# HanGuo97/flute

Hardware: AMD Instinct MI355X
Metric: qgemm effective GB/s, M=1, W4G64 NF4 fp16, K=N=4096 (Llama-3-8B linear), HBM-cold (higher is better)
Workload: dtype f16

## Files before the change

### flute_amd/csrc/qgemm_fast.h

```cpp
#pragma once
#include "qgemm_oneshot.h"

namespace flute_amd {

__host__ __device__ constexpr size_t fast_lds_bytes(int W, int KW, int D, int lg, int mb = 1) {
    return (size_t)65536 + (size_t)mb * 512 * D * KW * 2 + (size_t)W * 4 * D * (512 >> lg) * 2 + 128 + (size_t)W * 64;
}

struct FastRing { int R, GS; };
__host__ __device__ constexpr FastRing fast_ring_of(int opt) {
    constexpr FastRing rings[] = {{3, 8}, {2, 8}, {3, 8}, {4, 4}, {5, 4}, {3, 6}, {4, 5}};
    return rings[(opt >> 6) & 7];
}

template <typename T, int MB, int D, int R, int GS>
__device__ __forceinline__ void fast_pieces(ring16_t (&q)[D][1], uint32_t x_lane, uint32_t x_row, uint32_t s_lane, uint32_t s_piece,
                                            uint32_t lane_off, float (&acc)[4][MB]) {
    using NT = Num<T>;
    constexpr int NL = 16 * D;
    constexpr int NGR = (NL + GS - 1) / GS;
    static_assert(R >= 2 && GS >= 1 && GS <= 16, "lookup ring");
    auto younger = [](int g) constexpr {
        const int last = (g + R - 1 < NGR - 1) ? g + R - 1 : NGR - 1;
        const int end = ((last + 1) * GS < NL) ? (last + 1) * GS : NL;
        return end - (g + 1) * GS > 0 ? end - (g + 1) * GS : 0;
    };
    static_assert((R - 1) * GS <= 16, "at most one read of over-wait: lgkmcnt encodes 0 .. 15");
    ring16_t xq[D][MB];
    u32x2_t sq[D];
    uint32_t lv[NL];
    float al[4][MB];
#pragma unroll
    for (int i = 0; i < D; ++i)
#pragma unroll
        for (int m = 0; m < MB; ++m) xq[i][m] = lds_hidden128(x_lane + ((uint32_t)i << 10) + (uint32_t)m * x_row);
#pragma unroll
    for (int i = 0; i < D; ++i) sq[i] = lds_hidden64(s_lane + (uint32_t)i * s_piece);

    auto issue_group = [&](auto g_tag) {
        constexpr int g = decltype(g_tag)::value;
        constexpr int L0 = g * GS, L1 = (L0 + GS < NL) ? L0 + GS : NL;
        static_for<L1 - L0>([&](auto n_tag) {
            constexpr int L = L0 + decltype(n_tag)::value;
            if constexpr (L % 16 == 0) vm_wait_regs<D - 1 - L / 16>(q[L / 16][0]);
        });
        uint32_t ad[GS];
#pragma unroll
        for (int n = 0; n < L1 - L0; ++n) {
            const int L = L0 + n;
            ad[n] = __builtin_amdgcn_perm(q[L / 16][0][(L % 16) / 4], lane_off, 0x0c0c0400u | ((4u + (uint32_t)(L % 4)) << 8));
        }
#pragma unroll
        for (int n = 0; n < L1 - L0; ++n) { uint32_t& r = ad[n]; asm volatile("" : "+v"(r)); }
#pragma unroll
        for (int n = 0; n < L1 - L0; ++n) lv[L0 + n] = lds_lookup32(ad[n]);
    };
    auto wait_group = [&](auto g_tag) {
        constexpr int g = decltype(g_tag)::value;
        constexpr int L0 = g * GS, L1 = (L0 + GS < NL) ? L0 + GS : NL;
        constexpr int YOUNGER = younger(g);
        static_assert(YOUNGER <= 16, "over-wait");
        asm volatile("s_waitcnt lgkmcnt(%0)" : : "n"(YOUNGER < 15 ? YOUNGER : 15) : "memory");
#pragma unroll
        for (int n = L0; n < L1; ++n) { uint32_t& r = lv[n]; asm volatile("" : "+v"(r) : : "memory"); }
        if constexpr (g == 0) {
#pragma unroll
            for (int i = 0; i < D; ++i) {
#pragma unroll
                for (int m = 0; m < MB; ++m) { ring16_t& r = xq[i][m]; asm volatile("" : "+v"(r) : : "memory"); }
                u32x2_t& s2 = sq[i];
                asm volatile("" : "+v"(s2) : : "memory");
            }
        }
    };

    static_for<(R - 1 < NGR ? R - 1 : NGR)>([&](auto g_tag) { issue_group(g_tag); });
    static_for<NGR>([&](auto g_tag) {
        constexpr int g = decltype(g_tag)::value;
        constexpr int L0 = g * GS, L1 = (L0 + GS < NL) ? L0 + GS : NL;
        if constexpr (g + R - 1 < NGR) issue_group(std::integral_constant<int, g + R - 1>{});
        wait_group(g_tag);
#pragma unroll
        for (int L = L0; L < L1; ++L) {
            const int I = L / 16, ww = (L % 16) / 4, j = L % 4;
#pragma unroll
            for (int m = 0; m < MB; ++m) {
                if (ww == 0) al[j][m] = NT::dot2z(lv[L], xq[I][m][ww]);
                else al[j][m] = NT::dot2(lv[L], xq[I][m][ww], al[j][m]);
            }
            if (ww == 3) {
                const uint32_t w = sq[I][j / 2];
                const float sf = scale_to_float<T>((j & 1) ? (w >> 16) : (w & 0xffffu));
#pragma unroll
                for (int m = 0; m < MB; ++m) acc[j][m] = __builtin_fmaf(al[j][m], sf, acc[j][m]);
            }
        }
    });
}

template <typename T, int TILEP, int W, int KW, int D, int MB = 1, int OPT = 0>
__global__ __launch_bounds__(W * 64) void qgemv_fast_kernel(
    const uint32_t* __restrict__ Qp, const void* __restrict__ Sp, const void* __restrict__ Ap,
    const uint32_t* __restrict__ QM2, void* __restrict__ Dp, int N, int lg, int M,
    uint64_t* __restrict__ stamps) {
    using NT = Num<T>;
    constexpr int K = 512 * D * KW;
    constexpr bool POW2 = (D & (D - 1)) == 0;
    constexpr int LK = ilog2_c(K);
    constexpr int UPW = W / KW;
    constexpr int ENT = 256 / W;
    constexpr int RUNS = 32 / W;
    constexpr int XP = MB * K / 8;
    constexpr int XPR = (XP + W * 64 - 1) / (W * 64);
    constexpr int NSL = (2 * D * 8 + 63) / 64;
    constexpr uint32_t X_BASE = 65536u;
    constexpr uint32_t S_BASE = X_BASE + (uint32_t)MB * K * 2u;
    static_assert(W == 4 || W == 8 || W == 16, "waves per workgroup");
    static_assert(MB == 1 || MB == 2 || MB == 4, "rows per pass");
    static_assert((KW & (KW - 1)) == 0 && D >= 1 && D <= 8 && W % KW == 0, "K split: a power of two; 1 .. 8 pieces per wave");
    static_assert(MB * K * 2 <= 32768, "activation rows");

    extern __shared__ __attribute__((aligned(16))) char smem[];
    if (lds_base_of(smem) != 0) __builtin_trap();
#ifdef FLUTE_STAMPS
    uint64_t stamp[16];
    for (int i = 0; i < 16; ++i) stamp[i] = 0;
    stamp[0] = wall_clock64();
    stamp[1] = __builtin_amdgcn_s_memtime();
#define FLUTE_FSTAMP(i) stamp[i] = __builtin_amdgcn_s_memtime()
#else
#define FLUTE_FSTAMP(i)
#endif
    const int tid = threadIdx.x;
    const int lane = tid & 63;
    const int wave = __builtin_amdgcn_readfirstlane(tid >> 6);
    const uint32_t lane16 = (uint32_t)lane * 16u;
    const int gpp = 512 >> lg;
    const uint32_t red_base = S_BASE + (uint32_t)(W * 4 * D * gpp * 2);
    const int ul = wave / KW, kpart = wave % KW;
    const int unit = blockIdx.x * UPW + ul;
    const int col0 = (unit / TILEP) * (4 * TILEP) + (unit % TILEP);

    const srd_t lut_srd = make_srd(QM2, 1024u);
    uint32_t lut_v = buf_load4((uint32_t)(wave * ENT + (lane & (ENT - 1))) * 4u, lut_srd);
    const srd_t x_srd = make_srd(Ap, (uint32_t)M * (uint32_t)K * 2u);
    ring16_t xv[XPR];
#pragma unroll
    for (int r = 0; r < XPR; ++r) {
        const int pidx = (r * W + wave) * 64 + lane;
        xv[r] = buf_load16((XP % (W * 64) == 0 || pidx < XP) ? (uint32_t)pidx * 16u : 0x80000000u, x_srd, 0);
    }
    const int lgh = (8 + ilog2_c(D)) - lg;
    const int lG = LK - lg;
    const int G = K >> lg;
    const int gpw2 = (D * (512 >> lg)) >> 1;
    auto col_of = [&](int q) { return POW2 ? (q >> lgh) : (lg == 6 ? q / (D * 4) : (lg == 7 ? q / (D * 2) : q / D)); };
    const srd_t s_srd = make_srd(Sp, (uint32_t)((size_t)N * (size_t)G * 2));
    uint32_t sv[NSL];
#pragma unroll
    for (int r = 0; r < NSL; ++r) {
        const int q = lane + 64 * r;
        const int j = col_of(q);
        const int gp = POW2 ? (q & ((1 << lgh) - 1)) : (q - j * gpw2);
        const uint32_t vo = POW2 ? (uint32_t)((((col0 + j * TILEP) << lG) + (kpart << (lgh + 1)) + 2 * gp) * 2)
                                 : (uint32_t)(((col0 + j * TILEP) * G + kpart * 2 * gpw2 + 2 * gp) * 2);
        sv[r] = buf_load4_at(j < 4 ? vo : 0x80000000u, s_srd, 0);
    }
    const srd_t q_srd = make_srd(Qp + (size_t)unit * (K / 2), (uint32_t)K * 2u);
    ring16_t q[D][1];
    static_for<D>([&](auto i_tag) {
        constexpr int i = decltype(i_tag)::value;
        const uint32_t vo = lane16 + (uint32_t)(kpart * D + i) * 1024u;
        if constexpr (OPT & 1) q[i][0] = buf_load16(vo, q_srd, 0);
        else q[i][0] = buf_load16_nt(vo, q_srd, 0);
    });
    __builtin_amdgcn_sched_barrier(0);
    FLUTE_FSTAMP(2);

    vm_wait_regs<XPR + NSL + D>(lut_v);
    FLUTE_FSTAMP(3);
    {
        uint32_t te[RUNS];
#pragma unroll
        for (int u = 0; u < RUNS; ++u) te[u] = (uint32_t)__builtin_amdgcn_ds_bpermute((u * 8 + (lane >> 3)) * 4, (int)lut_v);
#pragma unroll
        for (int u = 0; u < RUNS; ++u) {
            const uint32_t addr = (uint32_t)(wave * ENT + u * 8 + (lane >> 3)) * 256u + (uint32_t)(lane & 7) * 16u;
            *reinterpret_cast<uint4*>(smem + addr) = make_uint4(te[u], te[u], te[u], te[u]);
        }
    }
    FLUTE_FSTAMP(4);
    if (KW > 1 && wave == 0 && lane < UPW) *reinterpret_cast<int*>(smem + red_base + lane * 4) = 0;
    static_for<XPR>([&](auto r_tag) {
        constexpr int r = decltype(r_tag)::value;
        vm_wait_regs<XPR - 1 - r + NSL + D>(xv[r]);
        if constexpr (r == 0) { FLUTE_FSTAMP(5); }
        const int pidx = (r * W + wave) * 64 + lane;
        if (XP % (W * 64) == 0 || pidx < XP) {
            *reinterpret_cast<uint4*>(smem + X_BASE + (uint32_t)pidx * 16u) = make_uint4(xv[r].x, xv[r].y, xv[r].z, xv[r].w);
        }
    });
    FLUTE_FSTAMP(6);
    asm volatile("s_waitcnt lgkmcnt(0)" ::: "memory");
    __builtin_amdgcn_s_barrier();
    FLUTE_FSTAMP(7);

    const uint32_t sbase = S_BASE + (uint32_t)(wave * 4 * D * gpp * 2);
#pragma unroll
    for (int r = 0; r < NSL; ++r) {
        vm_wait_regs<D>(sv[r]);
        const int qq = lane + 64 * r;
        const int j = col_of(qq);
        const int gp = POW2 ? (qq & ((1 << lgh) - 1)) : (qq - j * gpw2);
        if (j < 4) {
            uint16_t* img = reinterpret_cast<uint16_t*>(smem + sbase) + (2 * gp) * 4 + j;
            img[0] = (uint16_t)(sv[r] & 0xffffu);
            img[4] = (uint16_t)(sv[r] >> 16);
        }
    }
    FLUTE_FSTAMP(8);

    const uint32_t lane_off = (uint32_t)(lane & 31) * 4u;
    const int gl = (8 * lane) >> lg;
    const uint32_t s_lane = sbase + (uint32_t)(gl * 4) * 2u;
    const uint32_t x_lane = X_BASE + (uint32_t)(kpart * D * 64 + lane) * 16u;
    float acc[4][MB];
#pragma unroll
    for (int j = 0; j < 4; ++j)
#pragma unroll
        for (int m = 0; m < MB; ++m) acc[j][m] = 0.f;
    if constexpr (OPT & 2) {
        static_for<D>([&](auto i_tag) {
            constexpr int i = decltype(i_tag)::value;
            asm volatile("s_waitcnt vmcnt(%1)" : "+v"(q[i][0]) : "n"(D - 1 - i) : "memory");
#pragma unroll
            for (int ww = 0; ww < 4; ++ww) acc[ww][0] += __builtin_bit_cast(float, q[i][0][ww]);
        });
    } else {
        constexpr FastRing ring = fast_ring_of(OPT);
        fast_pieces<T, MB, D, ring.R, ring.GS>(q, x_lane, (uint32_t)K * 2u, s_lane, (uint32_t)(gpp * 4) * 2u, lane_off, acc);
    }
    FLUTE_FSTAMP(9);

    float v;
    int my_m;
    bool holder;
    transpose_reduce4<MB>(acc, lane, v, my_m, holder);
    FLUTE_FSTAMP(10);
    uint16_t* Dout = reinterpret_cast<uint16_t*>(Dp) + (size_t)my_m * N + col0 + (lane & 3) * TILEP;
    if constexpr (KW == 1) {
        if (holder && my_m < M) *Dout = NT::from_float(v);
    } else {
        const uint32_t rb = red_base + 128u;
        const uint32_t slot = (uint32_t)(my_m * 4 + (lane & 3)) * 4u;
        uint32_t ticket = 0;
        const uint32_t one = 1u;
        if (holder) {
            const uint32_t mine = rb + (uint32_t)wave * 64u + slot;
            asm volatile("ds_write_b32 %0, %1" : : "v"(mine), "v"(v) : "memory");
        }
        if (lane == 0) {
            const uint32_t tick = red_base + (uint32_t)ul * 4u;
            asm volatile("ds_add_rtn_u32 %0, %1, %2\n\ts_waitcnt lgkmcnt(0)" : "=&v"(ticket) : "v"(tick), "v"(one) : "memory");
        }
        const uint32_t t0 = (uint32_t)__builtin_amdgcn_readfirstlane((int)ticket);
        if (t0 == (uint32_t)(KW - 1) && holder && my_m < M) {
            float sum = 0.f;
#pragma unroll
            for (int kp = 0; kp < KW; ++kp) sum += __builtin_bit_cast(float, lds_ld32(rb + (uint32_t)(ul * KW + kp) * 64u + slot));
            *Dout = NT::from_float(sum);
        }
    }
#ifdef FLUTE_STAMPS
    FLUTE_FSTAMP(11);
    __builtin_amdgcn_s_waitcnt(0);
    stamp[12] = __builtin_amdgcn_s_memtime();
    stamp[13] = wall_clock64();
    if (lane == 0 && stamps != nullptr) {
        uint64_t* o = stamps + ((size_t)blockIdx.x * W + wave) * 16;
        for (int i = 0; i < 16; ++i) o[i] = stamp[i];
    }
#endif
#undef FLUTE_FSTAMP
}

}
```

Before: 2403.

## Reorder LDS lookup ring issue after wait and split weight load requests

Splits each lookup group's issue into an address-computation phase and an LDS-read phase. The next group's reads are now issued after the wait for the current group, so the lgkmcnt wait no longer has to account for the freshly issued reads. The default ring depth and group size change from (3,8) to (4,4). Only half of the quantized weight pieces are requested before the LUT wait; the rest are requested after it, so the first vmcnt wait covers fewer outstanding loads. The old ordering stays available behind an option bit. The risk is less overlap between LDS lookups and dot-product work, plus extra scheduling barriers.

```diff
diff --git a/flute_amd/csrc/qgemm_fast.h b/flute_amd/csrc/qgemm_fast.h
--- a/flute_amd/csrc/qgemm_fast.h
+++ b/flute_amd/csrc/qgemm_fast.h
@@ -9,11 +9,11 @@
 
 struct FastRing { int R, GS; };
 __host__ __device__ constexpr FastRing fast_ring_of(int opt) {
-    constexpr FastRing rings[] = {{3, 8}, {2, 8}, {3, 8}, {4, 4}, {5, 4}, {3, 6}, {4, 5}};
+    constexpr FastRing rings[] = {{4, 4}, {2, 8}, {3, 8}, {4, 4}, {5, 4}, {3, 6}, {4, 5}, {5, 3}};
     return rings[(opt >> 6) & 7];
 }
 
-template <typename T, int MB, int D, int R, int GS>
+template <typename T, int MB, int D, int R, int GS, bool OLD_ORDER = false>
 __device__ __forceinline__ void fast_pieces(ring16_t (&q)[D][1], uint32_t x_lane, uint32_t x_row, uint32_t s_lane, uint32_t s_piece,
                                             uint32_t lane_off, float (&acc)[4][MB]) {
     using NT = Num<T>;
@@ -37,14 +37,14 @@
 #pragma unroll
     for (int i = 0; i < D; ++i) sq[i] = lds_hidden64(s_lane + (uint32_t)i * s_piece);
 
-    auto issue_group = [&](auto g_tag) {
+    uint32_t ad[GS];
+    auto addr_group = [&](auto g_tag) {
         constexpr int g = decltype(g_tag)::value;
         constexpr int L0 = g * GS, L1 = (L0 + GS < NL) ? L0 + GS : NL;
         static_for<L1 - L0>([&](auto n_tag) {
             constexpr int L = L0 + decltype(n_tag)::value;
             if constexpr (L % 16 == 0) vm_wait_regs<D - 1 - L / 16>(q[L / 16][0]);
         });
-        uint32_t ad[GS];
 #pragma unroll
         for (int n = 0; n < L1 - L0; ++n) {
             const int L = L0 + n;
@@ -52,14 +52,20 @@
         }
 #pragma unroll
         for (int n = 0; n < L1 - L0; ++n) { uint32_t& r = ad[n]; asm volatile("" : "+v"(r)); }
+    };
+    auto read_group = [&](auto g_tag) {
+        constexpr int g = decltype(g_tag)::value;
+        constexpr int L0 = g * GS, L1 = (L0 + GS < NL) ? L0 + GS : NL;
 #pragma unroll
         for (int n = 0; n < L1 - L0; ++n) lv[L0 + n] = lds_lookup32(ad[n]);
     };
+    auto issue_group = [&](auto g_tag) { addr_group(g_tag); read_group(g_tag); };
     auto wait_group = [&](auto g_tag) {
         constexpr int g = decltype(g_tag)::value;
         constexpr int L0 = g * GS, L1 = (L0 + GS < NL) ? L0 + GS : NL;
-        constexpr int YOUNGER = younger(g);
-        static_assert(YOUNGER <= 16, "over-wait");
+        constexpr bool BEHIND = !OLD_ORDER && g + R - 1 < NGR;
+        constexpr int YOUNGER = younger(g) - (BEHIND ? ((g + R) * GS < NL ? GS : NL - (g + R - 1) * GS) : 0);
+        static_assert(YOUNGER >= 0 && YOUNGER <= 16, "over-wait");
         asm volatile("s_waitcnt lgkmcnt(%0)" : : "n"(YOUNGER < 15 ? YOUNGER : 15) : "memory");
 #pragma unroll
         for (int n = L0; n < L1; ++n) { uint32_t& r = lv[n]; asm volatile("" : "+v"(r) : : "memory"); }
@@ -78,8 +84,16 @@
     static_for<NGR>([&](auto g_tag) {
         constexpr int g = decltype(g_tag)::value;
         constexpr int L0 = g * GS, L1 = (L0 + GS < NL) ? L0 + GS : NL;
-        if constexpr (g + R - 1 < NGR) issue_group(std::integral_constant<int, g + R - 1>{});
-        wait_group(g_tag);
+        if constexpr (OLD_ORDER) {
+            if constexpr (g + R - 1 < NGR) issue_group(std::integral_constant<int, g + R - 1>{});
+            wait_group(g_tag);
+        } else {
+            if constexpr (g + R - 1 < NGR) addr_group(std::integral_constant<int, g + R - 1>{});
+            __builtin_amdgcn_sched_barrier(0);
+            wait_group(g_tag);
+            if constexpr (g + R - 1 < NGR) read_group(std::integral_constant<int, g + R - 1>{});
+            __builtin_amdgcn_sched_barrier(0);
+        }
 #pragma unroll
         for (int L = L0; L < L1; ++L) {
             const int I = L / 16, ww = (L % 16) / 4, j = L % 4;
@@ -168,17 +182,20 @@
     }
     const srd_t q_srd = make_srd(Qp + (size_t)unit * (K / 2), (uint32_t)K * 2u);
     ring16_t q[D][1];
-    static_for<D>([&](auto i_tag) {
+    constexpr int DQ0 = (OPT & 8) ? D : (D + 1) / 2;
+    auto request_piece = [&](auto i_tag) {
         constexpr int i = decltype(i_tag)::value;
         const uint32_t vo = lane16 + (uint32_t)(kpart * D + i) * 1024u;
         if constexpr (OPT & 1) q[i][0] = buf_load16(vo, q_srd, 0);
         else q[i][0] = buf_load16_nt(vo, q_srd, 0);
-    });
+    };
+    static_for<DQ0>(request_piece);
     __builtin_amdgcn_sched_barrier(0);
     FLUTE_FSTAMP(2);
 
-    vm_wait_regs<XPR + NSL + D>(lut_v);
+    vm_wait_regs<XPR + NSL + DQ0>(lut_v);
     FLUTE_FSTAMP(3);
+    static_for<D - DQ0>([&](auto i_tag) { request_piece(std::integral_constant<int, DQ0 + decltype(i_tag)::value>{}); });
     {
         uint32_t te[RUNS];
 #pragma unroll
@@ -238,7 +255,7 @@
         });
     } else {
         constexpr FastRing ring = fast_ring_of(OPT);
-        fast_pieces<T, MB, D, ring.R, ring.GS>(q, x_lane, (uint32_t)K * 2u, s_lane, (uint32_t)(gpp * 4) * 2u, lane_off, acc);
+        fast_pieces<T, MB, D, ring.R, ring.GS, (OPT & 4) != 0>(q, x_lane, (uint32_t)K * 2u, s_lane, (uint32_t)(gpp * 4) * 2u, lane_off, acc);
     }
     FLUTE_FSTAMP(9);
 
```

After: 2513 (median of 6 runs). 1.05x the previous value.
